# ZiyuanMa/R2D2

Hardware: AMD Instinct MI355X
Metric: learner seq-samples/sec (bs=64, L=80, 84x84x4 frames) (higher is better)
Workload: dtype bf16; 1 GPU; model=r2d2-nature-cnn-lstm512-dueling, global_batch=64, seq_len=80, burn_in=40, forward_steps=5, parallelism=dp1, engine=hip, replay=gpu-resident

## Files before the change

r2d2_amd/ops/engine.py:

```python

import os

import numpy as np
import torch

from .. import config as cfg
from ..models.encoders import ImpalaCNN, MLPEncoder
from . import hip_ops
from . import impala as impala_ops

PAD_HEAD = 32
KPAD = 32


def conv1_channels(encoder):
    return (1, 4) if encoder == "nature" else (4,)


MLP_WIDTH = 512
MLP_MAX_OBS = 16


def mlp_config_error(c):
    if c.hidden_dim != 512:
# ... 250 lines not shown
        self.online = _NetPack(online_net, self.device, self.A, with_bwd=True)
        self.target = _NetPack(target_net, self.device, self.A, with_bwd=False)
        self.online_net = online_net
        self.target_net = target_net
        self.bar = torch.zeros(512, dtype=torch.int32, device=self.device)
        self._empty = torch.Tensor()
        self._poison_pin = torch.zeros(2, dtype=torch.int32, pin_memory=True)

        params = [p for p in online_net.parameters()]
        n_total = sum(p.numel() for p in params)
        dev = self.device
        self.flat_param = torch.empty(n_total, dtype=torch.float32, device=dev)
        self.flat_grad = torch.zeros(n_total, dtype=torch.float32, device=dev)
        self.exp_avg = torch.zeros(n_total, dtype=torch.float32, device=dev)
        self.exp_avg_sq = torch.zeros(n_total, dtype=torch.float32, device=dev)
        self.norm_buf = torch.zeros(1, dtype=torch.float32, device=dev)
        self.adam_t = 0
        named = list(online_net.named_parameters())
        seg_of = lambda name: ("heads" if name.split(".")[0]
                               in ("advantage", "value")
                               else "lstm" if name.startswith("recurrent")
                               else "encoder")
        self.seg_ranges = {}
        ofs = 0
        for (name, _), p in zip(named, params):
            n = p.numel()
            self.flat_param[ofs:ofs + n].copy_(p.data.to(dev).view(-1))
            p.data = self.flat_param[ofs:ofs + n].view(p.shape)
            p.grad = self.flat_grad[ofs:ofs + n].view(p.shape)
            s = seg_of(name)
            lo, hi = self.seg_ranges.get(s, (ofs, ofs))
            assert hi == ofs, "segment params must be flat-contiguous"
            self.seg_ranges[s] = (min(lo, ofs), ofs + n)
            ofs += n
        self.timing = bool(os.environ.get("R2D2_ENGINE_TIMING"))
        self._events = []
        self.online.enable_fast_refresh(self.flat_param, self.m)
        self._graph = None
        self._graph_key = None
        self._use_graph = (os.environ.get("R2D2_HIP_GRAPH", "0") == "1"
                           and not self.timing and not self.mlp)

    def _mark(self, name):
        if self.timing:
            ev = torch.cuda.Event(enable_timing=True)
            ev.record()
            self._events.append((name, ev))

    def timing_report(self):
        torch.cuda.synchronize()
        out = []
        for (n0, e0), (n1, e1) in zip(self._events, self._events[1:]):
            out.append((n1, e0.elapsed_time(e1)))
        self._events.clear()
        return out

    def refresh_online(self):
        self.online.refresh()

    def optimizer_step(self, lr, eps, max_norm, betas=(0.9, 0.999)):
        self.adam_t += 1
        self.m.grad_sumsq(self.flat_grad, self.norm_buf)
        self.m.adam_step(self.flat_param, self.flat_grad, self.exp_avg,
                         self.exp_avg_sq, self.norm_buf, max_norm, lr,
                         betas[0], betas[1], eps, self.adam_t)

    def refresh_target(self):
        self.target.refresh()

    _fwd_band = os.environ.get("R2D2_CONV_FWD_BAND", "1") != "0"

    def _encoder_fwd(self, pack, obs_hwc_u8, want_stash=True):
        m = self.m
        if self.mlp:
            a1 = m.mlp_in_fwd(obs_hwc_u8, pack.mw1, pack.mb1)
            latent = m.gemm_bias_act(a1, pack.mw2t, pack.mb2, 1, False)
            return latent, (obs_hwc_u8, a1)
        if self.impala:
            return impala_ops.encoder_fwd(m, pack.imp, obs_hwc_u8, want_stash,
                                          xp=getattr(self, "_xp", None))
        M = obs_hwc_u8.shape[0]
        if self._fwd_band:
            a1 = m.conv_fwd_band(obs_hwc_u8, pack.w1t, pack.b1, 1, M)
            a2 = m.conv_fwd_band(a1, pack.w2t, pack.b2, 2, M)
            a3 = m.conv_fwd_band(a2, pack.w3t, pack.b3, 3, M)
        else:
            a1 = m.conv_fwd(obs_hwc_u8, pack.w1t, pack.b1, 1, M, 84, 84,
                            20, 20, True)
            a2 = m.conv_fwd(a1, pack.w2t, pack.b2, 2, M, 20, 20, 9, 9, True)
            a3 = m.conv_fwd(a2, pack.w3t, pack.b3, 3, M, 9, 9, 7, 7, True)
        flat = a3.view(M, 3136)
        latent = m.gemm_bias_act(flat, pack.wft, pack.bf, 1, False)
        return latent, (a1, a2, a3, flat)

    def _lstm_input(self, pack, latent, last_action, last_reward):
        M = latent.shape[0]
        rin = self.m.assemble_rin(
            latent.contiguous(),
            last_action.reshape(M, self.A).float().contiguous(),
            last_reward.reshape(M).float().contiguous(), pack.kin_pad)
        X = self.m.gemm_bias_act(rin, pack.wih_t, pack.lstm_bias, 0, False)
        return rin, X

    def _heads_fwd(self, pack, h):
        m = self.m
        adv1 = m.gemm_bias_act(h, pack.wa1t, pack.ba1, 1, False)
        adv2 = m.gemm_bias_act(adv1, pack.wa2t, pack.ba2, 0, True)
        val1 = m.gemm_bias_act(h, pack.wv1t, pack.bv1, 1, False)
        val2 = m.gemm_bias_act(val1, pack.wv2t, pack.bv2, 0, True)
        q = m.dueling_combine(adv2, val2, self.A)
        return q, (adv1, val1)

    _pos_cache = None

    def _positions(self, burn, learn, fwd, T):
        key = (T, burn.numpy().tobytes(), learn.numpy().tobytes(),
               fwd.numpy().tobytes())
        if self._pos_cache is None:
            self._pos_cache = {}
        if key in self._pos_cache:
            return self._pos_cache[key]
        n = self.cfg.forward_steps
        bu = burn.numpy().astype(np.int64)
        le = learn.numpy().astype(np.int64)
        fw = fwd.numpy().astype(np.int64)
        R = int(le.sum())
        b_of = np.repeat(np.arange(len(le), dtype=np.int64), le)
        starts = np.zeros(len(le), dtype=np.int64)
        starts[1:] = np.cumsum(le[:-1])
        within = np.arange(R, dtype=np.int64) - np.repeat(starts, le)
        t_learn = bu[b_of] + within
        t_tgt = np.minimum(t_learn + n, (bu + le + fw - 1)[b_of])
        dev = self.device
        lp = b_of * (T + 1) + t_learn + 1
        tp = b_of * (T + 1) + t_tgt + 1
        lbt = b_of * T + t_learn
        lp_t = torch.from_numpy(lp).to(dev)
        tp_t = torch.from_numpy(tp).to(dev)
        row_of = np.full(len(le) * T, -1, dtype=np.int32)
        row_of[lbt] = np.arange(R, dtype=np.int32)
        row_of_t = torch.from_numpy(row_of).to(dev)
        lens_dev = (burn + learn + fwd).to(torch.int32).to(dev)
        seg = torch.zeros(len(burn) + 1, dtype=torch.int32)
        seg[1:] = torch.cumsum(learn.to(torch.int32), 0)
        out = (lp_t, tp_t, row_of_t, lens_dev, seg.to(dev))
        if len(self._pos_cache) > 64:
            self._pos_cache.clear()
        self._pos_cache[key] = out
        return out

    def _layout_key(self, batch):
        return (tuple(batch.obs.shape), batch.obs.dtype,
                batch.burn_in_steps.numpy().tobytes(),
                batch.learning_steps.numpy().tobytes(),
                batch.forward_steps.numpy().tobytes())

    def _copy_into_static(self, batch):
        sb = self._static_batch
        for f in ("obs", "last_action", "last_reward", "hidden", "action",
                  "n_step_reward", "gamma", "is_weights"):
            getattr(sb, f).copy_(getattr(batch, f), non_blocking=True)

    def _try_capture(self, batch, key):
        import types
        dev = self.device
        sb = types.SimpleNamespace(
            obs=batch.obs.to(dev).contiguous().clone(),
            last_action=batch.last_action.to(dev).contiguous().clone(),
            last_reward=batch.last_reward.to(dev).contiguous().clone(),
            hidden=batch.hidden.to(dev).contiguous().clone(),
            action=batch.action.to(dev).contiguous().clone(),
            n_step_reward=batch.n_step_reward.to(dev).contiguous().clone(),
            gamma=batch.gamma.to(dev).contiguous().clone(),
            is_weights=batch.is_weights.to(dev).contiguous().clone(),
            burn_in_steps=batch.burn_in_steps,
            learning_steps=batch.learning_steps,
            forward_steps=batch.forward_steps)
        try:
            s = torch.cuda.Stream()
            s.wait_stream(torch.cuda.current_stream())
            with torch.cuda.stream(s):
                for _ in range(2):
                    self._train_step_impl(sb)
            torch.cuda.current_stream().wait_stream(s)
            g = torch.cuda.CUDAGraph()
            with torch.cuda.graph(g, capture_error_mode="thread_local"):
                loss, prio = self._train_step_impl(sb)
        except Exception as e:
            print(f"[engine] hipGraph capture failed ({e!r}); "
                  f"running uncaptured", flush=True)
            self._use_graph = False
            return False
        self._graph = g
        self._graph_key = key
        self._static_batch = sb
        self._graph_out = (loss, prio)
        return True

    def train_step(self, batch, grad_hook=None):
        check_batch_size(batch.obs.shape[0], "the batch's B")
        if bool(self._poison_pin.any()):
            raise RuntimeError(
                "persistent LSTM kernel poisoned on a previous step "
                "(bounded-spin timeout) — outputs/gradients of that step "
                "are invalid; aborting instead of training on them")
        if self._use_graph and grad_hook is None:
            key = self._layout_key(batch)
            if self._graph_key != key:
                self._try_capture(batch, key)
            if self._graph_key == key:
                self._copy_into_static(batch)
                self._graph.replay()
                return self._graph_out
        return self._train_step_impl(batch, grad_hook)

    def _train_step_impl(self, batch, grad_hook=None):
        m = self.m
        c = self.cfg
        dev = self.device
        B, T = batch.obs.shape[:2]
        A, H = self.A, self.H

        obs = batch.obs
        if self.mlp:
            if obs.dtype != torch.float32 or tuple(obs.shape[2:]) != (self.C,):
                raise TypeError(
                    f"the mlp encoder takes (B, T, {self.C}) float32 "
                    f"observations, got {tuple(obs.shape)} {obs.dtype}")
            obs_hwc = obs.reshape(B * T, self.C).contiguous()
        elif obs.shape[-1] == self.C and obs.shape[2] == 84:
            obs_hwc = obs.reshape(B * T, 84, 84, self.C)
        else:
            obs_hwc = obs.permute(0, 1, 3, 4, 2).reshape(B * T, 84, 84, self.C)
            obs_hwc = obs_hwc.contiguous()
        la = batch.last_action.to(dev)
        lr = batch.last_reward.to(dev)
        md = getattr(batch, "meta_dev", None)
        if md is not None:
            lp_t, tp_t, row_of, lens = m.positions_meta(
                md, batch.seg_dev, T, c.forward_steps,
                batch.action.shape[0], int(c.learning_steps))
            seg = batch.seg_dev
        else:
            lp_t, tp_t, row_of, lens, seg = self._positions(
                batch.burn_in_steps, batch.learning_steps,
                batch.forward_steps, T)
        R = lp_t.shape[0]
        init = batch.hidden.float().contiguous()

        self._mark("start")
        if self.impala:
            self._xp = impala_ops.pack_obs(m, self.online.imp, obs_hwc)
        lat_o, enc_stash = self._encoder_fwd(self.online, obs_hwc)
        self._mark("enc_online")
        lat_t, _ = self._encoder_fwd(self.target, obs_hwc, want_stash=False)
        self._mark("enc_target")
        rin_o, X_o = self._lstm_input(self.online, lat_o, la, lr)
        _, X_t = self._lstm_input(self.target, lat_t, la, lr)
        self._mark("lstm_input")
        Xo = X_o.view(B, T, 4 * H)
        Xt = X_t.view(B, T, 4 * H)
        lstm_fwd = m.lstm_fwd_multi if B > LSTM_SINGLE_ROWS else m.lstm_fwd
        Ho, Co, Ht, Ct, stash = lstm_fwd(
            Xo, Xt, self.online.whh_t, self.target.whh_t,
            init, init, lens, self.bar, True)
        self._poison_pin[0:1].copy_(self.bar[256:257], non_blocking=True)
        self._mark("lstm_fwd")

        Ho_flat = Ho.view(-1, H)
        h_learn = Ho_flat.index_select(0, lp_t)
        h_tgt_o = Ho_flat.index_select(0, tp_t)
        h_tgt_t = Ht.view(-1, H).index_select(0, tp_t)

        h_cat = torch.cat([h_learn, h_tgt_o], 0)
        q_cat, (adv1_o, val1_o) = self._heads_fwd(self.online, h_cat)
        q_learn, q_online_tgt = q_cat[:R], q_cat[R:]
        q_tgt, _ = self._heads_fwd(self.target, h_tgt_t)
        self._mark("heads")

        loss, dq, abs_td, _ = m.fused_double_q_loss(
            q_learn.contiguous(), q_online_tgt.contiguous(), q_tgt.contiguous(),
            batch.action.view(-1).long(), batch.n_step_reward, batch.gamma,
            batch.is_weights, c.rescale_eps, c.huber_kappa,
            0 if c.loss_fn == "mse" else 1)
        prio = m.segment_priority(abs_td, seg, c.prio_eta)
        self._mark("loss")

        ON = self.online
        net = self.online_net
        self.flat_grad.zero_()
        adv1_l, val1_l, h_l = adv1_o[:R], val1_o[:R], h_cat[:R]
        dadv2, dval2 = m.dueling_combine_bwd(dq.contiguous(),
                                             PAD_HEAD, PAD_HEAD)
        self._mark("hb_duel")
        dadv1 = m.gemm_dgrad(dadv2, self._empty, ON.wa2_kn, False)
        dh_a = m.gemm_dgrad(dadv1, adv1_l, ON.wa1_kn, True)
        dval1 = m.gemm_dgrad(dval2, self._empty, ON.wv2_kn, False)
        dh_v = m.gemm_dgrad(dval1, val1_l, ON.wv1_kn, True)
        self._mark("hb_dgrads")
        m.gemm_wgrad_into(dadv2, self._empty, adv1_l, False,
                          net.advantage[2].weight.grad,
                          net.advantage[2].bias.grad)
        m.gemm_wgrad_into(dadv1, adv1_l, h_l, True,
                          net.advantage[0].weight.grad,
                          net.advantage[0].bias.grad)
        m.gemm_wgrad_into(dval2, self._empty, val1_l, False,
                          net.value[2].weight.grad, net.value[2].bias.grad)
        m.gemm_wgrad_into(dval1, val1_l, h_l, True,
                          net.value[0].weight.grad, net.value[0].bias.grad)
        if grad_hook is not None:
            grad_hook("heads")
        self._mark("hb_wgrads")

        dHext = m.scatter_dh(dh_a, dh_v, row_of, B * T).view(B, T, H)
        self._mark("head_bwd")

        lstm_bwd = m.lstm_bwd_multi if B > LSTM_SINGLE_ROWS else m.lstm_bwd
        dgates = lstm_bwd(stash, Co, Ho, dHext.contiguous(), ON.whh_bwd,
                          lens, self.bar)
        self._poison_pin[1:2].copy_(self.bar[256:257], non_blocking=True)
        self._mark("lstm_bwd")
        dgates_flat = dgates.view(B * T, 4 * H)

        h_prev = Ho[:, :T].reshape(B * T, H).contiguous()
        m.gemm_wgrad_into(dgates_flat, self._empty, h_prev, False,
                          net.recurrent.weight_hh_l0.grad, self._empty)
        m.gemm_wgrad_into(dgates_flat, self._empty, rin_o, False,
                          net.recurrent.weight_ih_l0.grad,
                          net.recurrent.bias_ih_l0.grad)
        net.recurrent.bias_hh_l0.grad.copy_(net.recurrent.bias_ih_l0.grad)
        if grad_hook is not None:
            grad_hook("lstm")
        dlat = m.gemm_dgrad(dgates_flat, self._empty, ON.wih_kn, False, 512)
        self._mark("lstm_wgrads")

        M = B * T
        if self.mlp:
            X, a1 = enc_stash
            enc = net.encoder
# ... 162 lines not shown
```

r2d2_amd/ops/hip/bindings.cpp:

```cpp
#include <torch/extension.h>

#include <vector>

std::vector<torch::Tensor> fused_double_q_loss(
    torch::Tensor q_learn, torch::Tensor q_online_tgt, torch::Tensor q_target_tgt,
    torch::Tensor action, torch::Tensor n_step_reward, torch::Tensor gamma_n,
    torch::Tensor is_weights, double eps, double kappa, int64_t loss_kind);
torch::Tensor segment_priority(torch::Tensor abs_td, torch::Tensor seg_offsets,
                               double eta);

void sumtree_update(torch::Tensor tree, int64_t leaf_offset, torch::Tensor idxes,
                    torch::Tensor td, double alpha, int64_t old_ptr,
                    int64_t cur_ptr, int64_t seq_per_block, int64_t num_blocks);
std::vector<torch::Tensor> sumtree_sample(torch::Tensor tree, int64_t leaf_offset,
                                          int64_t num_levels, torch::Tensor jitter,
                                          int64_t n, double beta,
                                          int64_t max_idx);

std::vector<torch::Tensor> positions_meta(torch::Tensor meta, torch::Tensor seg,
                                          int64_t T, int64_t n, int64_t R,
                                          int64_t max_learn);
std::vector<torch::Tensor> replay_gather_meta(
    torch::Tensor idx, torch::Tensor burn_s, torch::Tensor learn_s,
    torch::Tensor fwd_s, torch::Tensor obs_start_s, torch::Tensor learn_off_s,
    int64_t spb);
std::vector<torch::Tensor> replay_gather_batch(
    torch::Tensor obs_store, torch::Tensor la_store, torch::Tensor lr_store,
    torch::Tensor act_store, torch::Tensor nsr_store, torch::Tensor gam_store,
    torch::Tensor hid_store, torch::Tensor idx, torch::Tensor meta,
    torch::Tensor seg, torch::Tensor weights, int64_t T, int64_t A,
    int64_t max_learn, int64_t H, int64_t spb);
std::vector<torch::Tensor> replay_gather_batch_dedup(
    torch::Tensor obs_store, torch::Tensor la_store, torch::Tensor lr_store,
    torch::Tensor act_store, torch::Tensor nsr_store, torch::Tensor gam_store,
    torch::Tensor hid_store, torch::Tensor idx, torch::Tensor meta,
    torch::Tensor seg, torch::Tensor weights, int64_t T, int64_t A,
    int64_t max_learn, int64_t H, int64_t spb, int64_t C);

torch::Tensor gemm_bias_act(torch::Tensor A, torch::Tensor Wt,
                            torch::Tensor bias, int64_t act, bool out_f32,
                            int64_t path);
torch::Tensor gemm_dgrad(torch::Tensor dY, torch::Tensor act_out,
                         torch::Tensor W, bool relu_mask, int64_t k_out,
                         c10::optional<torch::Tensor> out_mask, int64_t path);
std::vector<torch::Tensor> gemm_wgrad(torch::Tensor dY, torch::Tensor act_out,
                                      torch::Tensor A, bool relu_mask,
                                      bool want_bias, int64_t path);
void gemm_wgrad_into(torch::Tensor dY, torch::Tensor act_out, torch::Tensor A,
                     bool relu_mask, torch::Tensor dW_out,
                     torch::Tensor db_out,
                     int64_t kd0, int64_t kd1, int64_t kd2, int64_t path);

torch::Tensor conv_fwd(torch::Tensor in, torch::Tensor Wt, torch::Tensor bias,
                       int64_t conv_id, int64_t N, int64_t INH, int64_t INW,
                       int64_t OH, int64_t OW, bool relu);
torch::Tensor conv_dgrad_dense(torch::Tensor dY, torch::Tensor Wd,
                               torch::Tensor taps, torch::Tensor actx,
                               int64_t N, int64_t OH, int64_t OW, int64_t COUT,
                               int64_t XH, int64_t XW, int64_t CIN,
                               int64_t y0, int64_t x0, int64_t S,
                               torch::Tensor dX);
std::vector<torch::Tensor> conv_wgrad(torch::Tensor dY, torch::Tensor act,
                                      torch::Tensor in, int64_t conv_id,
                                      int64_t N, int64_t INH, int64_t INW,
                                      int64_t OH, int64_t OW, int64_t COUT,
                                      int64_t K);
std::vector<torch::Tensor> conv_wgrad_band(torch::Tensor dY, torch::Tensor act,
                                           torch::Tensor in, int64_t conv_id,
                                           int64_t N);
torch::Tensor conv_fwd_band(torch::Tensor in, torch::Tensor Wt,
                            torch::Tensor bias, int64_t conv_id, int64_t N,
                            int64_t max_wgs);
torch::Tensor conv_dgrad_band(torch::Tensor dY, torch::Tensor Wd,
                              torch::Tensor actx, int64_t conv_id, int64_t N,
                              int64_t max_wgs);

torch::Tensor assemble_rin(torch::Tensor latent, torch::Tensor la,
                           torch::Tensor lr, int64_t kin_pad);
void handoff_bench(torch::Tensor barrier_ws, int64_t steps, int64_t nblocks);
void handoff_payload_bench(torch::Tensor barrier_ws, torch::Tensor scratch,
                           int64_t steps, int64_t nblocks, int64_t kb,
                           int64_t mode);
void handoff_counter_bench(torch::Tensor barrier_ws, int64_t steps,
                           int64_t nblocks);
std::vector<torch::Tensor> lstm_fwd(
    torch::Tensor X0, torch::Tensor X1, torch::Tensor Whh0, torch::Tensor Whh1,
    torch::Tensor init0, torch::Tensor init1, torch::Tensor lens,
    torch::Tensor barrier_ws, bool want_stash);
torch::Tensor dueling_combine(torch::Tensor adv, torch::Tensor val, int64_t A);
torch::Tensor scatter_dh(torch::Tensor dh_a, torch::Tensor dh_v,
                         torch::Tensor row_of, int64_t BT);
std::vector<torch::Tensor> dueling_combine_bwd(torch::Tensor dq, int64_t PADA,
                                               int64_t PADV);
torch::Tensor lstm_bwd(torch::Tensor stash, torch::Tensor Cout,
                       torch::Tensor Hout, torch::Tensor dHext,
                       torch::Tensor Whh_bwd, torch::Tensor lens,
                       torch::Tensor barrier_ws);
std::vector<torch::Tensor> lstm_fwd_multi(
    torch::Tensor X0, torch::Tensor X1, torch::Tensor Whh0, torch::Tensor Whh1,
    torch::Tensor init0, torch::Tensor init1, torch::Tensor lens,
    torch::Tensor barrier_ws, bool want_stash, int64_t rows);
torch::Tensor lstm_bwd_multi(torch::Tensor stash, torch::Tensor Cout,
                             torch::Tensor Hout, torch::Tensor dHext,
                             torch::Tensor Whh_bwd, torch::Tensor lens,
                             torch::Tensor barrier_ws, int64_t rows);

void conv3p_pool(torch::Tensor in, torch::Tensor Wt, torch::Tensor bias,
                 torch::Tensor pout, torch::Tensor parg, int64_t N,
                 int64_t stage);
void conv3p(torch::Tensor in, torch::Tensor Wt, torch::Tensor bias,
            torch::Tensor res, torch::Tensor mask, torch::Tensor out,
            int64_t N, int64_t H, int64_t W, bool relu_in, bool has_bias,
            int64_t epi);
std::vector<torch::Tensor> conv3p_wgrad(torch::Tensor dY, torch::Tensor in,
                                        int64_t N, int64_t H, int64_t W,
                                        bool relu_in);
void maxpool3s2_fwd(torch::Tensor in, torch::Tensor out, torch::Tensor arg,
                    int64_t N, int64_t H, int64_t W);
void maxpool3s2_bwd(torch::Tensor dOut, torch::Tensor arg, torch::Tensor dIn,
                    int64_t N, int64_t H, int64_t W, int64_t OH, int64_t OW);
void pack_frames(torch::Tensor frames, torch::Tensor out, int64_t H,
                 int64_t W);
torch::Tensor pad2dense(torch::Tensor in, int64_t N, int64_t H, int64_t W,
                        bool relu);
void dense2pad_mask(torch::Tensor dflat, torch::Tensor act_pad,
                    torch::Tensor out, int64_t N, int64_t H, int64_t W);

void gather_pack(torch::Tensor flat, torch::Tensor m1, torch::Tensor m2,
                 torch::Tensor out);
torch::Tensor grad_sumsq(torch::Tensor grad, torch::Tensor norm_buf);
void adam_step(torch::Tensor param, torch::Tensor grad, torch::Tensor m,
               torch::Tensor v, torch::Tensor norm_buf, double max_norm,
               double lr, double beta1, double beta2, double eps,
               int64_t step);

void lstm_cell_step(torch::Tensor latent, torch::Tensor last_action,
                    torch::Tensor last_reward, torch::Tensor h0,
                    torch::Tensor c0, torch::Tensor wih_t,
                    torch::Tensor whh_t, torch::Tensor lstm_bias,
                    torch::Tensor h1, torch::Tensor c1, torch::Tensor hb,
                    int64_t units, int64_t rows);
void head_hidden_step(torch::Tensor hb, torch::Tensor wa1t, torch::Tensor ba1,
                      torch::Tensor wv1t, torch::Tensor bv1,
                      torch::Tensor adv1, torch::Tensor val1, int64_t rows);
void head_out_step(torch::Tensor adv1, torch::Tensor val1, torch::Tensor wa2t,
                   torch::Tensor ba2, torch::Tensor wv2t, torch::Tensor bv2,
                   torch::Tensor q, torch::Tensor greedy);

torch::Tensor mlp_in_fwd(torch::Tensor X, torch::Tensor W1, torch::Tensor b1);
void mlp_in_wgrad_into(torch::Tensor dA1, torch::Tensor X,
                       torch::Tensor dW1_out, torch::Tensor db1_out);

PYBIND11_MODULE(TORCH_EXTENSION_NAME, m) {
    m.doc() = "r2d2_amd gfx950 HIP kernels";
    m.def("fused_double_q_loss", &fused_double_q_loss,
          "Fused double-Q target + TD + loss + dLoss/dQ (returns loss, dq, "
          "abs_td, target)");
    m.def("segment_priority", &segment_priority,
          "Per-sequence mixed max/mean |TD| priority over ragged segments");
    m.def("sumtree_update", &sumtree_update,
          "GPU sum-tree priority update (duplicate-safe, ring-stale-masked)");
    m.def("sumtree_sample", &sumtree_sample,
          "GPU sum-tree stratified sample -> (idx, prio, is_weight)");
    m.def("replay_gather_meta", &replay_gather_meta,
          "Sampled-sequence metadata + segment offsets");
    m.def("positions_meta", &positions_meta,
          "engine gather/scatter position arrays from device-side sample "
          "metadata (no host round trip per ragged batch)");
    m.def("replay_gather_batch", &replay_gather_batch,
          "On-device padded batch assembly from the GPU block store");
    m.def("replay_gather_batch_dedup", &replay_gather_batch_dedup,
          "replay_gather_batch from the frame-once store: one (H, W) frame "
          "per step, obs_rows + C - 1 frames per slot; the (B, T, H*W*C) HWC "
          "stacks are rebuilt in the gather");
    m.def("gemm_bias_act", &gemm_bias_act, "MFMA GEMM + bias + activation",
          pybind11::arg("A"), pybind11::arg("Wt"), pybind11::arg("bias"),
          pybind11::arg("act"), pybind11::arg("out_f32"),
          pybind11::arg("path") = 0);
    m.def("gemm_dgrad", &gemm_dgrad,
          "MFMA GEMM backward-data (+ fused ReLU mask; optional dense "
          "k_out-column output; optional fused output ReLU mask)",
          pybind11::arg("dY"), pybind11::arg("act_out"), pybind11::arg("W"),
          pybind11::arg("relu_mask"), pybind11::arg("k_out") = 0,
          pybind11::arg("out_mask") = pybind11::none(),
          pybind11::arg("path") = 0);
    m.def("gemm_wgrad", &gemm_wgrad, "MFMA GEMM backward-weight (+ bias grad)",
          pybind11::arg("dY"), pybind11::arg("act_out"), pybind11::arg("A"),
          pybind11::arg("relu_mask"), pybind11::arg("want_bias"),
          pybind11::arg("path") = 0);
    m.def("gemm_wgrad_into", &gemm_wgrad_into,
          "GEMM backward-weight accumulated straight into .grad views "
          "(optional (d0,d1,d2)->(d2,d0,d1) k-axis store permutation)",
          pybind11::arg("dY"), pybind11::arg("act_out"), pybind11::arg("A"),
          pybind11::arg("relu_mask"), pybind11::arg("dW_out"),
          pybind11::arg("db_out"), pybind11::arg("kd0") = 0,
          pybind11::arg("kd1") = 0, pybind11::arg("kd2") = 0,
          pybind11::arg("path") = 0);
    m.def("conv_fwd", &conv_fwd, "Implicit-GEMM MFMA conv forward (NHWC)");
    m.def("conv_dgrad_dense", &conv_dgrad_dense,
          "MFMA conv backward-data from dense pre-masked dY (bounds-checked "
          "taps, optional fused output ReLU mask)");
    m.def("scatter_dh", &scatter_dh,
          "dHext (BT, H) from head-backward rows via inverse position map");
    m.def("conv_wgrad", &conv_wgrad, "MFMA conv backward-weight");
    m.def("conv_wgrad_band", &conv_wgrad_band,
          "per-image band wgrad (whole input image LDS-staged, one dequant "
          "per element, register accumulation, one atomic flush per wg)");
    m.def("conv_fwd_band", &conv_fwd_band,
          "per-image band forward (image LDS-resident; weights in LDS for "
          "conv1, in registers for the 64-output layers)",
          py::arg("in"), py::arg("Wt"), py::arg("bias"), py::arg("conv_id"),
          py::arg("N"), py::arg("max_wgs") = 0);
    m.def("conv_dgrad_band", &conv_dgrad_band,
          "per-image band dgrad: dY staged once in LDS in a zero halo, all "
          "parity classes in one launch, dX stored through LDS with the "
          "optional fused output ReLU mask",
          py::arg("dY"), py::arg("Wd"), py::arg("actx"), py::arg("conv_id"),
          py::arg("N"), py::arg("max_wgs") = 0);
    m.def("lstm_fwd", &lstm_fwd,
          "Persistent fused LSTM forward (dual-network, length-masked)");
    m.def("lstm_bwd", &lstm_bwd, "Persistent fused LSTM BPTT backward");
    m.def("lstm_fwd_multi", &lstm_fwd_multi,
          "Persistent fused LSTM forward for 1 <= B <= 256: one launch, "
          "passes of `rows` (64 or 128; 0 = R2D2_LSTM_MULTI_ROWS / default) "
          "batch rows with W_hh LDS-resident across passes",
          py::arg("X0"), py::arg("X1"), py::arg("Whh0"), py::arg("Whh1"),
          py::arg("init0"), py::arg("init1"), py::arg("lens"),
          py::arg("barrier_ws"), py::arg("want_stash"), py::arg("rows") = 0);
    m.def("lstm_bwd_multi", &lstm_bwd_multi,
          "Persistent fused LSTM BPTT backward for 1 <= B <= 256 (multi-pass)",
          py::arg("stash"), py::arg("Cout"), py::arg("Hout"),
          py::arg("dHext"), py::arg("Whh_bwd"), py::arg("lens"),
          py::arg("barrier_ws"), py::arg("rows") = 0);
    m.def("assemble_rin", &assemble_rin,
          "fused LSTM-input row assembly (latent | action | reward | pad)");
    m.def("handoff_bench", &handoff_bench, "producer-flag handoff microbench");
    m.def("handoff_payload_bench", &handoff_payload_bench,
          "counter handoff behind kb KB of stores per block: mode 0 plain "
          "stores + release fence, mode 1 sc1 stores, no fence");
    m.def("handoff_counter_bench", &handoff_counter_bench,
          "counter-aggregated handoff microbench");
    m.def("dueling_combine", &dueling_combine, "q = V + A - mean(A)");
    m.def("dueling_combine_bwd", &dueling_combine_bwd, "dueling combine backward");
    m.def("conv3p", &conv3p,
          "IMPALA 3x3 s1 p1 conv on halo-padded NHWC (fwd & dgrad-as-conv, "
          "fused relu-in / residual / mask epilogues)");
    m.def("conv3p_pool", &conv3p_pool,
          "IMPALA stage conv FUSED with maxpool 3x3 s2 (conv output stays "
          "in LDS; emits pooled activations + tap argmax)");
    m.def("conv3p_wgrad", &conv3p_wgrad,
          "IMPALA 3x3 conv backward-weight (padded dY, relu-in patches)");
    m.def("maxpool3s2_fwd", &maxpool3s2_fwd,
          "maxpool 3x3 s2 p1 forward + tap argmax");
    m.def("maxpool3s2_bwd", &maxpool3s2_bwd,
          "maxpool backward (atomic-free input-side gather)");
    m.def("pack_frames", &pack_frames,
          "u8 HWC frames -> halo-padded 8-channel u8");
    m.def("pad2dense", &pad2dense, "padded NHWC -> dense rows (+relu)");
    m.def("dense2pad_mask", &dense2pad_mask,
          "dense grad -> padded, masked by act>0 (relu backward)");
    m.def("lstm_cell_step", &lstm_cell_step,
          "fused single-step LSTM cell for actor inference: input-row "
          "assembly, both gate GEMMs, bias, nonlinearities and cell update "
          "in one launch; writes h1, c1 (f32) and hb = bf16(h1)",
          py::arg("latent"), py::arg("last_action"), py::arg("last_reward"),
          py::arg("h0"), py::arg("c0"), py::arg("wih_t"), py::arg("whh_t"),
          py::arg("lstm_bias"), py::arg("h1"), py::arg("c1"), py::arg("hb"),
          py::arg("units") = 0, py::arg("rows") = 0);
    m.def("head_hidden_step", &head_hidden_step,
          "both dueling-head 512 -> 512 ReLU hidden layers in one launch",
          py::arg("hb"), py::arg("wa1t"), py::arg("ba1"), py::arg("wv1t"),
          py::arg("bv1"), py::arg("adv1"), py::arg("val1"),
          py::arg("rows") = 0);
    m.def("head_out_step", &head_out_step,
          "both dueling-head output layers + q = V + A - mean(A) + greedy "
          "action (first index of the row maximum) in one launch");
    m.def("mlp_in_fwd", &mlp_in_fwd,
          "MLP encoder first layer: A1 (M, 512) bf16 = relu(X (M, D) f32 . "
          "W1 (512, D)^T + b1), 1 <= D <= 16, f32 accumulation",
          py::arg("X"), py::arg("W1"), py::arg("b1"));
    m.def("mlp_in_wgrad_into", &mlp_in_wgrad_into,
          "MLP encoder first-layer weight gradient accumulated into .grad "
          "views: dW1 (512, D) += dA1^T . X, db1 (512,) += column sums of "
          "dA1 (bf16, already ReLU-masked)",
          py::arg("dA1"), py::arg("X"), py::arg("dW1_out"),
          py::arg("db1_out"));
    m.def("gather_pack", &gather_pack,
          "regenerate prepacked weights from the flat param buffer "
          "(index-map gather, one launch per dtype)");
    m.def("grad_sumsq", &grad_sumsq, "flat gradient squared-norm reduction");
    m.def("adam_step", &adam_step,
          "fused multi-tensor clip + Adam on the flat parameter buffer");
}
```

r2d2_amd/ops/hip/conv_kernels.hip:

```cpp

#include <hip/hip_runtime.h>
#include <torch/extension.h>
#include <ATen/cuda/CUDAContext.h>

#include "common.h"

__device__ __forceinline__ bf16x8 dequant8(unsigned lo, unsigned hi) {
    bf16x8 r;
    const float inv = 1.f / 255.f;
#pragma unroll
    for (int i = 0; i < 4; ++i)
        r[i] = (__bf16)(((lo >> (8 * i)) & 0xff) * inv);
#pragma unroll
    for (int i = 0; i < 4; ++i)
        r[4 + i] = (__bf16)(((hi >> (8 * i)) & 0xff) * inv);
    return r;
}

__device__ __forceinline__ bf16x8 load_dequant8(const unsigned char* p) {
    uint2 raw = *reinterpret_cast<const uint2*>(p);
    return dequant8(raw.x, raw.y);
}

template <int CIN>
// ... 556 lines not shown
            }
        }
    }
    tile.flush(dWt, db, reinterpret_cast<float*>(s_dy));
}

template <int KSTEPS>
__device__ __forceinline__ void load_b_regs(bf16x8 (&b)[KSTEPS][2],
                                            const __hip_bfloat16* W, int col0,
                                            int lane) {
    const __hip_bfloat16* p =
        W + (long)(col0 + (lane & 15)) * (KSTEPS * 32) + (lane >> 4) * 8;
#pragma unroll
    for (int ks = 0; ks < KSTEPS; ++ks)
#pragma unroll
        for (int j = 0; j < 2; ++j)
            b[ks][j] = load_bf16x8(p + (long)j * 16 * (KSTEPS * 32) + ks * 32);
}

template <class G>
__global__ __launch_bounds__(256, 2) void conv_fwd_band64_kernel(
    const void* __restrict__ in,
    const __hip_bfloat16* __restrict__ Wt,
    const float* __restrict__ bias,
    __hip_bfloat16* __restrict__ out,
    int N, int imgs_per_wg) {
    using Img = GatherImage<G>;
    constexpr int K = G::K, NPIX = G::NPIX, KSTEPS = K / 32;
    constexpr int NI = ((NPIX + 15) / 16 + 1) / 2;
    static_assert(G::COUT == 64 && !G::IN_U8 && G::CIN % 32 == 0);
    __shared__ __attribute__((aligned(16))) __hip_bfloat16 s_img[Img::SIZE];

    const int wave = threadIdx.x / WAVE, lane = threadIdx.x & (WAVE - 1);
    const int wr = wave >> 1, col0 = (wave & 1) * 32;
    const int frow = lane & 15, kseg = (lane >> 4) * 8;

    bf16x8 b[KSTEPS][2];
    load_b_regs<KSTEPS>(b, Wt, col0, lane);
    float bias_c[2];
#pragma unroll
    for (int j = 0; j < 2; ++j) bias_c[j] = bias[col0 + j * 16 + frow];

    int pbase[NI];
#pragma unroll
    for (int i = 0; i < NI; ++i) {
        int pp = min((wr * NI + i) * 16 + frow, NPIX - 1);
        pbase[i] = (pp / G::OW * Img::RS + pp % G::OW * Img::PS) * G::S + kseg;
    }

    const long n0 = (long)blockIdx.x * imgs_per_wg;
    const long n1 = min((long)N, n0 + imgs_per_wg);
    for (long n = n0; n < n1; ++n) {
        __syncthreads();
        stage_image<G, Img>(s_img, in, n);
        __syncthreads();

        f32x4 acc[NI][2] = {};
#pragma unroll
        for (int ks = 0; ks < KSTEPS; ++ks) {
            constexpr int CIN = G::CIN;
            const int rem = ks * 32 % G::KWC;
            const int off = ks * 32 / G::KWC * Img::RS + rem / CIN * Img::PS
                            + rem % CIN;
            bf16x8 a[NI];
#pragma unroll
            for (int i = 0; i < NI; ++i)
                a[i] = *reinterpret_cast<const bf16x8*>(
                    &s_img[pbase[i] + off]);
#pragma unroll
            for (int i = 0; i < NI; ++i)
#pragma unroll
                for (int j = 0; j < 2; ++j)
                    acc[i][j] = __builtin_amdgcn_mfma_f32_16x16x32_bf16(
                        a[i], b[ks][j], acc[i][j], 0, 0, 0);
        }
        for_each_acc(acc, lane, [&](int r, int c, float v) {
            int pp = wr * NI * 16 + r;
            if (pp < NPIX) {
                v += bias_c[c / 16];
                out[(n * NPIX + pp) * G::COUT + col0 + c] =
                    f2bf(fmaxf(v, 0.f));
            }
        });
    }
}

template <class G>
struct DgradBand {
    static constexpr int S = G::S, NCLS = S * S;
    static constexpr int TH = G::KH / S, TW = G::KW / S;
    static constexpr int HY = TH - 1, HX = TW - 1;
    static constexpr int SH = G::OH + 2 * HY, SW = G::OW + 2 * HX;
    static constexpr int PS = G::COUT + 16;
    static constexpr int RS = NCLS == 1 ? 976 : 928;
    static constexpr int DY_SIZE = SH * RS;
    static constexpr int PSX = G::CIN + 8;
    static constexpr int DX_SIZE = G::INH * G::INW * PSX;
    static constexpr int K = G::TAPS * G::COUT, KSTEPS = K / 32;
    static constexpr int NROWS = G::CLS_H * G::CLS_W;
    static constexpr int NFRAG = (NROWS + 15) / 16;
    static constexpr int NI = NCLS == 1 ? (NFRAG + 1) / 2 : NFRAG;
    static constexpr int DY_CHUNKS = G::NPIX * G::COUT / 8;
    static constexpr int DX_CHUNKS = G::IMG / 8;
    static constexpr int NDY = (DY_CHUNKS + 255) / 256;
    static constexpr int NDX = (DX_CHUNKS + 255) / 256;
    static_assert(G::COUT == 64 && RS >= SW * PS && RS % 8 == 0);
    static_assert((NCLS == 1 && G::CIN == 64) || (NCLS == 4 && G::CIN == 32),
                  "wave split: 2x2 over 64 columns, or one class per wave");
    static_assert((DY_SIZE + DX_SIZE) * 2 <= 64 * 1024);
};

template <class G, bool OUT_MASK>
__global__ __launch_bounds__(256, 2) void conv_dgrad_band_kernel(
    const __hip_bfloat16* __restrict__ dY,
    const __hip_bfloat16* __restrict__ Wd,
    const __hip_bfloat16* __restrict__ actx,
    __hip_bfloat16* __restrict__ dX,
    int N, int imgs_per_wg) {
    using D = DgradBand<G>;
    constexpr int COUT = G::COUT, CIN = G::CIN;
    __shared__ __attribute__((aligned(16))) __hip_bfloat16 s_dy[D::DY_SIZE];
    __shared__ __attribute__((aligned(16))) __hip_bfloat16 s_dx[D::DX_SIZE];

    const int wave = threadIdx.x / WAVE, lane = threadIdx.x & (WAVE - 1);
    const int cls = D::NCLS == 1 ? 0 : wave;
    const int frag0 = D::NCLS == 1 ? (wave >> 1) * D::NI : 0;
    const int col0 = D::NCLS == 1 ? (wave & 1) * 32 : 0;
    const int py = cls / G::S, px = cls % G::S;
    const int frow = lane & 15, kseg = (lane >> 4) * 8;

    bf16x8 b[D::KSTEPS][2];
    load_b_regs<D::KSTEPS>(b, Wd + (long)cls * CIN * D::K, col0, lane);

    int abase[D::NI];
#pragma unroll
    for (int i = 0; i < D::NI; ++i) {
        int q = min((frag0 + i) * 16 + frow, D::NROWS - 1);
        abase[i] = (q / G::CLS_W + D::HY) * D::RS
                   + (q % G::CLS_W + D::HX) * D::PS + kseg;
    }
    int dyoff[D::NDY];
#pragma unroll
    for (int c = 0; c < D::NDY; ++c) {
        int e8 = min((int)threadIdx.x + c * 256, D::DY_CHUNKS - 1);
        int pix = e8 / (COUT / 8);
        dyoff[c] = (pix / G::OW + D::HY) * D::RS
                   + (pix % G::OW + D::HX) * D::PS + e8 % (COUT / 8) * 8;
    }
    auto load_dy = [&](bf16x8 (&pre)[D::NDY], long n) {
        const __hip_bfloat16* g = dY + n * (G::NPIX * COUT);
#pragma unroll
        for (int c = 0; c < D::NDY; ++c) {
            int e8 = threadIdx.x + c * 256;
            if (e8 < D::DY_CHUNKS) pre[c] = load_bf16x8(g + e8 * 8);
        }
    };

    const long n0 = (long)blockIdx.x * imgs_per_wg;
    const long n1 = min((long)N, n0 + imgs_per_wg);
    if (n0 >= n1) return;
    bf16x8 pre[D::NDY];
    load_dy(pre, n0);
    for (int e = threadIdx.x * 8; e < D::DY_SIZE; e += 256 * 8)
        *reinterpret_cast<bf16x8*>(&s_dy[e]) = zero_bf16x8();
    __syncthreads();

// ... 186 lines not shown
    auto launch = [&](auto kernel) {
        hipLaunchKernelGGL(
            kernel, grid, dim3(256), 0,
            at::cuda::getCurrentCUDAStream().stream(),
            reinterpret_cast<const __hip_bfloat16*>(dY.data_ptr()),
            reinterpret_cast<const __hip_bfloat16*>(Wd.data_ptr()),
            has_m ? reinterpret_cast<const __hip_bfloat16*>(actx.data_ptr())
                  : nullptr,
            reinterpret_cast<__hip_bfloat16*>(dX.data_ptr()),
            taps.data_ptr<int>(), (int)Mc, (int)y0, (int)x0);
    };
    if (has_m) launch(conv_dgrad_dense_kernel<G, true>);
    else launch(conv_dgrad_dense_kernel<G, false>);
}

torch::Tensor conv_dgrad_dense(torch::Tensor dY, torch::Tensor Wd,
                               torch::Tensor taps, torch::Tensor actx,
                               int64_t N, int64_t OH, int64_t OW, int64_t COUT,
                               int64_t XH, int64_t XW, int64_t CIN,
                               int64_t y0, int64_t x0, int64_t S,
                               torch::Tensor dX) {
    if (dgrad_dense_is<Conv3>(OH, OW, COUT, XH, XW, CIN, S))
        dgrad_dense_launch<Conv3>(dY, Wd, taps, actx, N, y0, x0, dX);
    else if (dgrad_dense_is<Conv2>(OH, OW, COUT, XH, XW, CIN, S))
        dgrad_dense_launch<Conv2>(dY, Wd, taps, actx, N, y0, x0, dX);
    else
        TORCH_CHECK(false, "conv_dgrad_dense: only conv3 (", Conv3::OH, "x",
                    Conv3::OW, "x", Conv3::COUT, " -> ", Conv3::INH, "x",
                    Conv3::INW, "x", Conv3::CIN, ", stride ", Conv3::S,
                    ") and conv2 (", Conv2::OH, "x", Conv2::OW, "x",
                    Conv2::COUT, " -> ", Conv2::INH, "x", Conv2::INW, "x",
                    Conv2::CIN, ", stride ", Conv2::S,
                    ") are instantiated; got ", OH, "x", OW, "x", COUT, " -> ",
                    XH, "x", XW, "x", CIN, ", stride ", S);
    return dX;
}

static void band_grid(int64_t N, int64_t wgs, int& imgs, int& grid) {
    imgs = cdiv(N, std::max<int64_t>(1, wgs));
    grid = cdiv(N, imgs);
}

torch::Tensor conv_fwd_band(torch::Tensor in, torch::Tensor Wt,
                            torch::Tensor bias, int64_t conv_id, int64_t N,
                            int64_t max_wgs) {
    const char* who = "conv_fwd_band";
    torch::Tensor out;
    TORCH_CHECK(N > 0 && max_wgs >= 0, who, ": N must be positive and max_wgs "
                "non-negative");
    int cin1 = conv1_cin(conv_id, in, N, 8, 8, who);
    dispatch_layer(conv_id, cin1, who, [&](auto g) {
        using G = decltype(g);
        check_weights<G>(Wt, who);
        check_input<G>(in, N, who);
        TORCH_CHECK(Wt.is_cuda() && Wt.dtype() == torch::kBFloat16
                    && Wt.is_contiguous()
                    && reinterpret_cast<uintptr_t>(Wt.data_ptr()) % 16 == 0
                    && bias.is_cuda() && bias.dtype() == torch::kFloat32
                    && bias.is_contiguous() && bias.numel() == G::COUT, who,
                    ": weights must be contiguous, 16-byte aligned bf16 and "
                    "bias ", G::COUT, " f32, both on the device");
        out = torch::empty({N * G::NPIX, G::COUT},
                           in.options().dtype(torch::kBFloat16));
        int imgs, grid;
        auto stream = at::cuda::getCurrentCUDAStream().stream();
        auto wt = reinterpret_cast<const __hip_bfloat16*>(Wt.data_ptr());
        auto op = reinterpret_cast<__hip_bfloat16*>(out.data_ptr());
        if constexpr (G::COUT == 64) {
            band_grid(N, max_wgs > 0 ? max_wgs : BAND_WGS, imgs, grid);
            hipLaunchKernelGGL(
                (conv_fwd_band64_kernel<G>), dim3(grid), dim3(256), 0, stream,
                in.data_ptr(), wt, bias.data_ptr<float>(), op, (int)N, imgs);
        } else {
            band_grid(N, max_wgs > 0 ? max_wgs : (G::CIN == 1 ? 2048 : BAND_WGS),
                      imgs, grid);
            for (int co0 = 0; co0 < G::COUT; co0 += BAND_COLS)
                hipLaunchKernelGGL(
                    (conv_fwd_band_kernel<G>), dim3(grid), dim3(256), 0,
                    stream, in.data_ptr(), wt, bias.data_ptr<float>(), op,
                    (int)N, imgs, co0);
        }
    });
    return out;
}

torch::Tensor conv_dgrad_band(torch::Tensor dY, torch::Tensor Wd,
                              torch::Tensor actx, int64_t conv_id, int64_t N,
                              int64_t max_wgs) {
    const char* who = "conv_dgrad_band";
    torch::Tensor dX;
    TORCH_CHECK(conv_id == 2 || conv_id == 3, who,
                ": only conv2 and conv3 have a dgrad, got conv_id ", conv_id);
    TORCH_CHECK(N > 0 && max_wgs >= 0, who, ": N must be positive and max_wgs "
                "non-negative");
    dispatch_layer(conv_id, 0, who, [&](auto g) {
        using G = decltype(g);
        if constexpr (!G::IN_U8) {
            using D = DgradBand<G>;
            bool has_m = actx.defined() && actx.numel() > 0;
            TORCH_CHECK(dY.numel() == N * G::NPIX * G::COUT, who,
                        ": dY must hold N*", G::NPIX * G::COUT, " elements");
            TORCH_CHECK(Wd.dim() >= 2 && Wd.numel() == D::NCLS * G::CIN * D::K
                        && Wd.size(-1) == D::K && Wd.size(-2) == G::CIN, who,
                        ": Wd must be (", D::NCLS, ", ", G::CIN, ", ", D::K,
                        "), got ", Wd.sizes());
            if (has_m)
                TORCH_CHECK(actx.numel() == N * G::IMG, who,
                            ": the mask must hold N*", G::IMG, " elements");
            for (const torch::Tensor* t : {&dY, &Wd, &actx})
                TORCH_CHECK((t == &actx && !has_m)
                            || (t->is_cuda() && t->dtype() == torch::kBFloat16
                                && t->is_contiguous()
                                && reinterpret_cast<uintptr_t>(t->data_ptr())
                                       % 16 == 0), who,
                            ": dY, Wd and the mask must be contiguous, 16-byte "
                            "aligned bf16 device tensors");
            dX = torch::empty({N, G::INH, G::INW, G::CIN}, dY.options());
            int imgs, grid;
            band_grid(N, max_wgs > 0 ? max_wgs : BAND_WGS, imgs, grid);
            auto launch = [&](auto kernel) {
                hipLaunchKernelGGL(
                    kernel, dim3(grid), dim3(256), 0,
                    at::cuda::getCurrentCUDAStream().stream(),
                    reinterpret_cast<const __hip_bfloat16*>(dY.data_ptr()),
                    reinterpret_cast<const __hip_bfloat16*>(Wd.data_ptr()),
                    has_m ? reinterpret_cast<const __hip_bfloat16*>(
                                actx.data_ptr()) : nullptr,
                    reinterpret_cast<__hip_bfloat16*>(dX.data_ptr()), (int)N,
                    imgs);
            };
            if (has_m) launch(conv_dgrad_band_kernel<G, true>);
            else launch(conv_dgrad_band_kernel<G, false>);
        }
    });
    return dX;
}

std::vector<torch::Tensor> conv_wgrad_band(torch::Tensor dY, torch::Tensor act,
                                           torch::Tensor in, int64_t conv_id,
                                           int64_t N) {
    const char* who = "conv_wgrad_band";
    torch::Tensor dWt, db;
    int cin1 = conv1_cin(conv_id, in, N, 8, 8, who);
    dispatch_layer(conv_id, cin1, who, [&](auto g) {
        using G = decltype(g);
        check_input<G>(in, N, who);
        check_grads<G>(dY, act, N, who);
        dWt =
            torch::zeros({G::COUT, G::K}, dY.options().dtype(torch::kFloat32));
        db = torch::zeros({G::COUT}, dY.options().dtype(torch::kFloat32));
        int imgs = cdiv(N, 512);
        int grid = cdiv(N, imgs);
        hipLaunchKernelGGL(
            (conv_wgrad_band_kernel<G>), dim3(grid), dim3(256), 0,
            at::cuda::getCurrentCUDAStream().stream(),
            reinterpret_cast<const __hip_bfloat16*>(dY.data_ptr()),
            reinterpret_cast<const __hip_bfloat16*>(act.data_ptr()),
            in.data_ptr(), dWt.data_ptr<float>(), db.data_ptr<float>(), (int)N,
            imgs);
    });
    return {dWt, db};
}

std::vector<torch::Tensor> conv_wgrad(torch::Tensor dY, torch::Tensor act,
                                      torch::Tensor in, int64_t conv_id,
                                      int64_t N, int64_t INH, int64_t INW,
// ... 29 lines not shown
```

Before: 21730 seq/s.

## Fuse online and target conv1 forward into one dual-weight kernel

Adds a conv1 forward kernel that stages and dequantizes each uint8 frame into LDS once and computes conv1 for both the online and target networks. Both weight sets stay in registers, and outputs go through per-wave LDS scratch so they can be written with 16-byte stores. The engine now runs this dual kernel and then finishes conv2/conv3 for each network separately. This removes one full read and dequantize of the observation batch and one kernel launch. In exchange it uses more registers and LDS per workgroup, which may lower occupancy, and both conv1 outputs are alive at once, which raises peak memory.

```diff
diff --git a/r2d2_amd/ops/engine.py b/r2d2_amd/ops/engine.py
--- a/r2d2_amd/ops/engine.py
+++ b/r2d2_amd/ops/engine.py
@@ -356,11 +356,18 @@
         M = obs_hwc_u8.shape[0]
         if self._fwd_band:
             a1 = m.conv_fwd_band(obs_hwc_u8, pack.w1t, pack.b1, 1, M)
+        else:
+            a1 = m.conv_fwd(obs_hwc_u8, pack.w1t, pack.b1, 1, M, 84, 84,
+                            20, 20, True)
+        return self._encoder_from_a1(pack, a1)
+
+    def _encoder_from_a1(self, pack, a1):
+        m = self.m
+        M = a1.shape[0] // 400
+        if self._fwd_band:
             a2 = m.conv_fwd_band(a1, pack.w2t, pack.b2, 2, M)
             a3 = m.conv_fwd_band(a2, pack.w3t, pack.b3, 3, M)
         else:
-            a1 = m.conv_fwd(obs_hwc_u8, pack.w1t, pack.b1, 1, M, 84, 84,
-                            20, 20, True)
             a2 = m.conv_fwd(a1, pack.w2t, pack.b2, 2, M, 20, 20, 9, 9, True)
             a3 = m.conv_fwd(a2, pack.w3t, pack.b3, 3, M, 9, 9, 7, 7, True)
         flat = a3.view(M, 3136)
@@ -525,10 +532,22 @@
         self._mark("start")
         if self.impala:
             self._xp = impala_ops.pack_obs(m, self.online.imp, obs_hwc)
-        lat_o, enc_stash = self._encoder_fwd(self.online, obs_hwc)
-        self._mark("enc_online")
-        lat_t, _ = self._encoder_fwd(self.target, obs_hwc, want_stash=False)
-        self._mark("enc_target")
+        if self._fwd_band and not (self.mlp or self.impala):
+            a1_o, a1_t = m.conv1_fwd_dual(
+                obs_hwc, self.online.w1t, self.online.b1, self.target.w1t,
+                self.target.b1, B * T)
+            self._mark("conv1_dual")
+            lat_o, enc_stash = self._encoder_from_a1(self.online, a1_o)
+            self._mark("enc_online")
+            lat_t, _ = self._encoder_from_a1(self.target, a1_t)
+            del a1_t
+            self._mark("enc_target")
+        else:
+            lat_o, enc_stash = self._encoder_fwd(self.online, obs_hwc)
+            self._mark("enc_online")
+            lat_t, _ = self._encoder_fwd(self.target, obs_hwc,
+                                         want_stash=False)
+            self._mark("enc_target")
         rin_o, X_o = self._lstm_input(self.online, lat_o, la, lr)
         _, X_t = self._lstm_input(self.target, lat_t, la, lr)
         self._mark("lstm_input")
diff --git a/r2d2_amd/ops/hip/bindings.cpp b/r2d2_amd/ops/hip/bindings.cpp
--- a/r2d2_amd/ops/hip/bindings.cpp
+++ b/r2d2_amd/ops/hip/bindings.cpp
@@ -71,6 +71,11 @@
 torch::Tensor conv_fwd_band(torch::Tensor in, torch::Tensor Wt,
                             torch::Tensor bias, int64_t conv_id, int64_t N,
                             int64_t max_wgs);
+std::vector<torch::Tensor> conv1_fwd_dual(torch::Tensor in, torch::Tensor Wt0,
+                                          torch::Tensor bias0,
+                                          torch::Tensor Wt1,
+                                          torch::Tensor bias1, int64_t N,
+                                          int64_t max_wgs);
 torch::Tensor conv_dgrad_band(torch::Tensor dY, torch::Tensor Wd,
                               torch::Tensor actx, int64_t conv_id, int64_t N,
                               int64_t max_wgs);
@@ -211,6 +216,11 @@
           "conv1, in registers for the 64-output layers)",
           py::arg("in"), py::arg("Wt"), py::arg("bias"), py::arg("conv_id"),
           py::arg("N"), py::arg("max_wgs") = 0);
+    m.def("conv1_fwd_dual", &conv1_fwd_dual,
+          "conv1 of two networks from one LDS staging of each frame (both "
+          "weight sets in registers, 16-byte stores); returns (out0, out1)",
+          py::arg("in"), py::arg("Wt0"), py::arg("bias0"), py::arg("Wt1"),
+          py::arg("bias1"), py::arg("N"), py::arg("max_wgs") = 0);
     m.def("conv_dgrad_band", &conv_dgrad_band,
           "per-image band dgrad: dY staged once in LDS in a zero halo, all "
           "parity classes in one launch, dX stored through LDS with the "
diff --git a/r2d2_amd/ops/hip/conv_kernels.hip b/r2d2_amd/ops/hip/conv_kernels.hip
--- a/r2d2_amd/ops/hip/conv_kernels.hip
+++ b/r2d2_amd/ops/hip/conv_kernels.hip
@@ -662,6 +662,133 @@
                     f2bf(fmaxf(v, 0.f));
             }
         });
+    }
+}
+
+template <class G>
+struct Conv1Dual {
+    static constexpr int CHUNKS = G::IMG / 8;
+    static constexpr int NPRE = (CHUNKS + 255) / 256;
+    static constexpr int NFRAG = G::NPIX / 16;
+    static constexpr int PER_WAVE = NFRAG / 4;
+    static constexpr int SCR_LD = G::COUT + 8;
+    static constexpr int SCR = 32 * SCR_LD;
+    static constexpr int KS_STEP = 32 / G::KWC * G::INW * G::CIN;
+    static_assert(G::NPIX % 16 == 0 && NFRAG % 4 == 1 && PER_WAVE % 2 == 0,
+                  "whole fragments: pairs per wave, wave 0 one single more");
+    static_assert(G::COUT == 32 && G::IN_U8 && 32 % G::KWC == 0);
+    static_assert((G::IMG + 4 * SCR) * 2 <= 80 * 1024);
+};
+
+template <class G>
+__global__ __launch_bounds__(256, 2) void conv1_fwd_dual_kernel(
+    const unsigned char* __restrict__ in,
+    const __hip_bfloat16* __restrict__ Wt0,
+    const float* __restrict__ bias0,
+    const __hip_bfloat16* __restrict__ Wt1,
+    const float* __restrict__ bias1,
+    __hip_bfloat16* __restrict__ out0,
+    __hip_bfloat16* __restrict__ out1,
+    int N, int imgs_per_wg) {
+    using D = Conv1Dual<G>;
+    constexpr int NPIX = G::NPIX, COUT = G::COUT, KSTEPS = G::K / 32;
+    __shared__ __attribute__((aligned(16))) __hip_bfloat16 s_img[G::IMG];
+    __shared__ __attribute__((aligned(16))) __hip_bfloat16 s_scr[4 * D::SCR];
+
+    const int wave = threadIdx.x / WAVE, lane = threadIdx.x & (WAVE - 1);
+    const int frow = lane & 15, kseg = (lane >> 4) * 8;
+    __hip_bfloat16* scr = s_scr + wave * D::SCR;
+
+    bf16x8 b[2][KSTEPS][2];
+    load_b_regs<KSTEPS>(b[0], Wt0, 0, lane);
+    load_b_regs<KSTEPS>(b[1], Wt1, 0, lane);
+    float bias_c[2][2];
+#pragma unroll
+    for (int j = 0; j < 2; ++j) {
+        bias_c[0][j] = bias0[j * 16 + frow];
+        bias_c[1][j] = bias1[j * 16 + frow];
+    }
+    const int klane = kseg / G::KWC * G::INW * G::CIN + kseg % G::KWC;
+
+    auto load_image = [&](uint2 (&pre)[D::NPRE], long n) {
+        const uint2* g = reinterpret_cast<const uint2*>(in + n * G::IMG);
+#pragma unroll
+        for (int c = 0; c < D::NPRE; ++c) {
+            int e8 = threadIdx.x + c * 256;
+            if (e8 < D::CHUNKS) pre[c] = g[e8];
+        }
+    };
+
+    auto tile = [&](auto ni, int f0, long n) {
+        constexpr int NI = decltype(ni)::value;
+        int pbase[NI];
+#pragma unroll
+        for (int i = 0; i < NI; ++i) {
+            int pp = (f0 + i) * 16 + frow;
+            pbase[i] = (pp / G::OW * G::INW + pp % G::OW) * G::S * G::CIN
+                       + klane;
+        }
+        f32x4 acc[2][NI][2] = {};
+#pragma unroll
+        for (int ks = 0; ks < KSTEPS; ++ks) {
+            bf16x8 a[NI];
+#pragma unroll
+            for (int i = 0; i < NI; ++i)
+                a[i] = lds_patch_row<G::CIN>(
+                    &s_img[pbase[i] + ks * D::KS_STEP]);
+#pragma unroll
+            for (int q = 0; q < 2; ++q)
+#pragma unroll
+                for (int i = 0; i < NI; ++i)
+#pragma unroll
+                    for (int j = 0; j < 2; ++j)
+                        acc[q][i][j] = __builtin_amdgcn_mfma_f32_16x16x32_bf16(
+                            a[i], b[q][ks][j], acc[q][i][j], 0, 0, 0);
+        }
+#pragma unroll
+        for (int q = 0; q < 2; ++q) {
+            for_each_acc(acc[q], lane, [&](int r, int c, float v) {
+                v += bias_c[q][c / 16];
+                scr[r * D::SCR_LD + c] = f2bf(fmaxf(v, 0.f));
+            });
+            __builtin_amdgcn_fence(__ATOMIC_RELEASE, "wavefront");
+            __builtin_amdgcn_wave_barrier();
+            __builtin_amdgcn_fence(__ATOMIC_ACQUIRE, "wavefront");
+            __hip_bfloat16* go =
+                (q ? out1 : out0) + (n * NPIX + f0 * 16) * COUT + lane * 8;
+#pragma unroll
+            for (int i = 0; i < NI; ++i)
+                *reinterpret_cast<bf16x8*>(go + i * 16 * COUT) =
+                    *reinterpret_cast<const bf16x8*>(
+                        &scr[(i * 16 + lane / 4) * D::SCR_LD + lane % 4 * 8]);
+            __builtin_amdgcn_fence(__ATOMIC_RELEASE, "wavefront");
+            __builtin_amdgcn_wave_barrier();
+            __builtin_amdgcn_fence(__ATOMIC_ACQUIRE, "wavefront");
+        }
+    };
+
+    const long n0 = (long)blockIdx.x * imgs_per_wg;
+    const long n1 = min((long)N, n0 + imgs_per_wg);
+    if (n0 >= n1) return;
+    const int f0 = wave == 0 ? 0 : 1 + wave * D::PER_WAVE;
+    uint2 pre[D::NPRE];
+    load_image(pre, n0);
+    for (long n = n0; n < n1; ++n) {
+        __syncthreads();
+#pragma unroll
+        for (int c = 0; c < D::NPRE; ++c) {
+            int e8 = threadIdx.x + c * 256;
+            if (e8 < D::CHUNKS)
+                *reinterpret_cast<bf16x8*>(&s_img[e8 * 8]) =
+                    dequant8(pre[c].x, pre[c].y);
+        }
+        __syncthreads();
+        if (n + 1 < n1) load_image(pre, n + 1);
+
+        for (int t = 0; t < D::PER_WAVE; t += 2)
+            tile(std::integral_constant<int, 2>{}, f0 + t, n);
+        if (wave == 0)
+            tile(std::integral_constant<int, 1>{}, D::PER_WAVE, n);
     }
 }
 
@@ -1014,6 +1141,57 @@
         }
     });
     return out;
+}
+
+constexpr int DUAL_WGS_4CH = 512, DUAL_WGS_1CH = 2048;
+
+std::vector<torch::Tensor> conv1_fwd_dual(torch::Tensor in, torch::Tensor Wt0,
+                                          torch::Tensor bias0,
+                                          torch::Tensor Wt1,
+                                          torch::Tensor bias1, int64_t N,
+                                          int64_t max_wgs) {
+    const char* who = "conv1_fwd_dual";
+    torch::Tensor out0, out1;
+    TORCH_CHECK(N > 0 && max_wgs >= 0, who, ": N must be positive and max_wgs "
+                "non-negative");
+    int cin1 = conv1_cin(1, in, N, 8, 8, who);
+    dispatch_layer(1, cin1, who, [&](auto g) {
+        using G = decltype(g);
+        if constexpr (G::IN_U8) {
+            for (const torch::Tensor* w : {&Wt0, &Wt1}) {
+                TORCH_CHECK(w->is_cuda() && w->dtype() == torch::kBFloat16
+                            && w->is_contiguous()
+                            && reinterpret_cast<uintptr_t>(w->data_ptr()) % 16
+                                   == 0, who, ": weights must be contiguous, "
+                            "16-byte aligned bf16 device tensors");
+                check_weights<G>(*w, who);
+            }
+            for (const torch::Tensor* b : {&bias0, &bias1})
+                TORCH_CHECK(b->is_cuda() && b->dtype() == torch::kFloat32
+                            && b->is_contiguous() && b->numel() == G::COUT,
+                            who, ": each bias must be ", G::COUT,
+                            " contiguous f32 on the device");
+            auto opts = in.options().dtype(torch::kBFloat16);
+            out0 = torch::empty({N * G::NPIX, G::COUT}, opts);
+            out1 = torch::empty({N * G::NPIX, G::COUT}, opts);
+            int imgs, grid;
+            band_grid(N, max_wgs > 0 ? max_wgs
+                         : (G::CIN == 1 ? DUAL_WGS_1CH : DUAL_WGS_4CH),
+                      imgs, grid);
+            hipLaunchKernelGGL(
+                (conv1_fwd_dual_kernel<G>), dim3(grid), dim3(256), 0,
+                at::cuda::getCurrentCUDAStream().stream(),
+                reinterpret_cast<const unsigned char*>(in.data_ptr()),
+                reinterpret_cast<const __hip_bfloat16*>(Wt0.data_ptr()),
+                bias0.data_ptr<float>(),
+                reinterpret_cast<const __hip_bfloat16*>(Wt1.data_ptr()),
+                bias1.data_ptr<float>(),
+                reinterpret_cast<__hip_bfloat16*>(out0.data_ptr()),
+                reinterpret_cast<__hip_bfloat16*>(out1.data_ptr()), (int)N,
+                imgs);
+        }
+    });
+    return {out0, out1};
 }
 
 torch::Tensor conv_dgrad_band(torch::Tensor dY, torch::Tensor Wd,
```

Result: faster. 23410 seq/s (median of 6 runs) (+7.7%).
